# kolinko/effort

Measured on NVIDIA H100. Metric: Mistral-7B decode tok/s @ effort 0.25, higher is better.
Workload: dtype fp16 weights, f32 accumulate

## Files before the change

effort_b200/build.py:

```python
from __future__ import annotations

import os
import shutil
import subprocess

HERE = os.path.dirname(os.path.abspath(__file__))
CSRC = os.path.join(HERE, "csrc")
LIB = os.path.join(HERE, "libeffort_b200.so")
SOURCES = ["effort_capi.cu", "safetensors_io.cpp"]
HEADERS = ["common.cuh", "cutoff.cuh", "bucket_mul.cuh", "convert.cuh", "q4.cuh", "decode.cuh", "comm.cuh"]
NVCC_FLAGS = [
    "-gencode", "arch=compute_90a,code=sm_90a", "-O3", "-lineinfo", "-std=c++17",
    "-Xcompiler", "-fPIC", "-shared",
]


def _nvcc() -> str:
    for cand in (os.environ.get("NVCC"), shutil.which("nvcc"), "/usr/local/cuda/bin/nvcc"):
        if cand and os.path.exists(cand):
            return cand
    raise RuntimeError("nvcc not found: the effort_b200 CUDA extension cannot be built")


def needs_build() -> bool:
    if not os.path.exists(LIB):
        return True
    t = os.path.getmtime(LIB)
    deps = [os.path.join(CSRC, s) for s in SOURCES + HEADERS] + [os.path.join(HERE, "..", "include", "effort_b200.h")]
    return any(os.path.exists(d) and os.path.getmtime(d) > t for d in deps)


def build(force: bool = False, verbose: bool = False) -> str:
    if not force and not needs_build():
        return LIB
    extra = os.environ.get("EFFORT_NVCC_EXTRA", "").split()
    cmd = [_nvcc()] + NVCC_FLAGS + extra + (["-Xptxas", "-v"] if verbose else []) + ["-o", LIB] + \
          [os.path.join(CSRC, s) for s in SOURCES]
    host_cc = "/usr/bin/g++"
    if os.path.exists(host_cc):
        cmd += ["-ccbin", host_cc]
    r = subprocess.run(cmd, capture_output=True, text=True)
    if r.returncode != 0:
        raise RuntimeError("nvcc failed:\n" + r.stdout + r.stderr)
# ... 8 lines not shown
```

effort_b200/csrc/bucket_mul_v2.cuh:

```cuda
#pragma once
#include "bucket_mul.cuh"

namespace effort {

constexpr int kV2Warps = 16;
constexpr int kV2Threads = kV2Warps * 32;
constexpr int kUnitRows = 4;
template <int VEC> struct V2Unit {
    static constexpr int kRowStride = 32 * VEC * 2;
    static constexpr int kUnitBytes = kUnitRows * kRowStride + 32;
};
constexpr int kV2MaxInputs = kV2Threads;

enum VMode : int { kVPlain = 0, kVNorm = 1, kVSilu = 2 };
enum OutMode : int { kOutOverwrite = 0, kOutAccumulate = 1 };
enum CutMode : int { kCutSelect = 0, kCutBisect = 1 };

struct V2Problem {
    const float* v;
    const float* v2;
    const float* v_cut;
    const __half* norm_w;
    const __half* st16;
    const float* st32;
    const uint16_t* bk;
    const __half* probes;
    const uint32_t* exp_no;
    float* out;
    const float* out_scale;
    unsigned* sync;
    uint32_t* sel_counts;
    float* cutoff_out;
    float* cutoff_hint;
    int* rounds_out;
    unsigned* err_flag;
    unsigned long long* trace;
    float4* red_part;
    unsigned* red_sync;
    unsigned long long* unit_trace;
    float norm_eps;
    int in, C, P, q, layout, out_mode;
    int CS, RS, W;
    int R, lpr;
};

struct V2Batch {
    int n;
    int list_cap;
    int dynamic;
    int ring_bytes;
    int prefetch;
    int lookahead;
    int trace_cycles;
    int window;
    int cta_begin[kMulBatchMax + 1];
    V2Problem p[kMulBatchMax];
};

struct V2Header {
    CutoffSmem cut;
    unsigned sel_acc[8][2];
    float red[kV2Warps];
    int warp_cnt[kV2Warps];
    int warp_rows[kV2Warps];
    int next_unit;
};

template <int SLOTS, int VEC>
struct V2Smem {
    static constexpr int kTileFloats = SLOTS * 32 * VEC;
    static constexpr int kTileBytes = kTileFloats * 4;
    static constexpr size_t kHdrBytes = (sizeof(V2Header) + 127) & ~size_t(127);
    static __host__ __device__ size_t list_bytes(int cap) { return ((size_t)cap * 2 + 127) & ~size_t(127); }
    static constexpr size_t kStatBytes = SLOTS == 16 ? 0 : (size_t)kV2MaxInputs * 8 * 4;
    static constexpr int kUnitsPerInput = SLOTS == 16 ? 8 : 4;
    static __host__ __device__ size_t fixed_bytes(int cap) {
        return (size_t)kTileBytes + (size_t)kV2Warps * kTileBytes + kHdrBytes + 2 * (size_t)kV2MaxInputs * 4 + kStatBytes +
               list_bytes(cap) + 128;
    }
    static __host__ __device__ size_t bytes(int cap, int ring_units) {
        return fixed_bytes(cap) + (size_t)kV2Warps * ring_units * V2Unit<VEC>::kUnitBytes;
    }
};

__device__ __forceinline__ void cp_async16(uint32_t dst, const void* src, uint64_t pol) {
    asm volatile("cp.async.cg.shared.global.L2::cache_hint [%0], [%1], 16, %2;" ::"r"(dst), "l"(src), "l"(pol) : "memory");
}
// ... 536 lines not shown
```

effort_b200/csrc/bucket_mul_v4.cuh:

```cuda
#pragma once
#include "bucket_mul_v3.cuh"

namespace effort {

constexpr int kV4Pairs = 8;
constexpr int kV4Units = 16;
constexpr int kV4RingBytes = 16 * 1024;
constexpr int kV4SelWarps = 8;
constexpr int kSelVals = EFFORT_PROBES_MAX / (kV4SelWarps * 32);
constexpr int kSelKeys = kSelVals / 2, kSelChunks = kSelVals / 8;
static_assert(kSelVals * kV4SelWarps * 32 == EFFORT_PROBES_MAX && kSelChunks >= 1, "the group holds all 4096 products");

struct __align__(16) V4Desc {
    uint32_t off;
    uint32_t n;
    float val;
    uint32_t charged;
};

struct V4Header {
    CutoffSmem cut;
    uint2 sel_slot[2][kV4SelWarps];
    float red[kV4SelWarps];
    float cutoff, denom;
    int sel_rows;
    uint32_t warp_rows[kV2Threads / 32];
    uint32_t start[kV4Pairs + 1];
    unsigned long long full_bar[kV4Pairs][kV4Units];
    unsigned long long empty_bar[kV4Pairs][kV4Units];
    V4Desc desc[kV4Pairs][kV4Units];
};

struct V4Smem {
    static constexpr int kTileFloats = 16 * 32 * 4;
    static constexpr int kTileBytes = kTileFloats * 4;
    static constexpr size_t kHdrBytes = (sizeof(V4Header) + 127) & ~size_t(127);
    static constexpr size_t kBytes = (size_t)kTileBytes  + (size_t)kV4Pairs * kTileBytes + kHdrBytes +
                                     (size_t)kV2MaxInputs * 16 + 128 + (size_t)kV4Pairs * kV4RingBytes +
                                     1024 ;
};

__device__ __forceinline__ void cp_async_arrive_noinc(uint32_t bar) {
    asm volatile("cp.async.mbarrier.arrive.noinc.shared::cta.b64 [%0];" ::"r"(bar) : "memory");
}

__device__ __forceinline__ bool mbar_wait_parked(uint32_t bar, uint32_t parity) {
    uint32_t done = 0;
    for (int tries = 0; tries < (1 << 22) && !done; tries++) {
        asm volatile("{ .reg .pred p; mbarrier.try_wait.parity.shared::cta.b64 p, [%1], %2, %3; selp.u32 %0, 1, 0, p; }"
                     : "=r"(done) : "r"(bar), "r"(parity), "r"(200u) : "memory");
    }
    return done != 0;
}

__device__ __forceinline__ bool mbar_test(uint32_t bar, uint32_t parity) {
    uint32_t done;
    asm volatile("{ .reg .pred p; mbarrier.test_wait.parity.shared::cta.b64 p, [%1], %2; selp.u32 %0, 1, 0, p; }"
                 : "=r"(done) : "r"(bar), "r"(parity) : "memory");
    return done != 0;
}

__device__ __forceinline__ float div_by(float x, float d, float r) {
    const float q = x * r;
    return fmaf(fmaf(-q, d, x), r, q);
}

__device__ __forceinline__ uint32_t count_gt32(const uint32_t (&keys)[kSelKeys], uint32_t th) {
    const __nv_bfloat162 t = as_bf162(splat_bf16(th));
    __nv_bfloat162 c0 = __hgt2(as_bf162(keys[0]), t), c1 = __hgt2(as_bf162(keys[1]), t);
#pragma unroll
    for (int i = 2; i < kSelKeys; i += 2) {
        c0 = __hadd2(c0, __hgt2(as_bf162(keys[i]), t));
        c1 = __hadd2(c1, __hgt2(as_bf162(keys[i + 1]), t));
// ... 90 lines not shown
    for (int rho = 0; rho < 16; rho++) sel_stat[rho] = 0.f;
    auto load_stats = [&](int j, float (&st)[16]) {
        const int i = rsp + j * RS;
        if (P == 16) {
            const uint4* sp = reinterpret_cast<const uint4*>(pb.st16 + ((size_t)e_no * pb.in + i) * 16);
            const uint4 a = ldg_keep_u4(sp, keep), b = ldg_keep_u4(sp + 1, keep);
            const uint32_t ws[8] = {a.x, a.y, a.z, a.w, b.x, b.y, b.z, b.w};
#pragma unroll
            for (int q2 = 0; q2 < 8; q2++) {
                const float2 f = __half22float2(*reinterpret_cast<const __half2*>(&ws[q2]));
                st[2 * q2] = f.x;
                st[2 * q2 + 1] = f.y;
            }
        } else {
#pragma unroll
            for (int rho = 0; rho < 16; rho++)
                if (rho < P) st[rho] = __half2float(pb.st16[((size_t)e_no * pb.in + i) * P + rho]);
        }
    };
    if (tid < n_in) load_stats(tid, sel_stat);
    const int vmode = pb.norm_w ? kVNorm : (pb.v2 ? kVSilu : kVPlain);
    uint4 prb[kSelChunks], nwv[kSelChunks];
    if (CUT == kCutSelect && sel_warp) {
        const uint4* pp = reinterpret_cast<const uint4*>(pb.probes + (size_t)e_no * EFFORT_PROBES_MAX) + kSelChunks * tid;
#pragma unroll
        for (int c = 0; c < kSelChunks; c++) prb[c] = ldg_keep_u4(pp + c, keep);
        if (vmode == kVNorm) {
            const uint4* np4 = reinterpret_cast<const uint4*>(pb.norm_w) + kSelChunks * tid;
#pragma unroll
            for (int c = 0; c < kSelChunks; c++) nwv[c] = np4[c];
        }
    }
    if (warp == NC) {
        for (int s = lane; s < NC * kV4Units; s += 32) {
            mbar_init((uint32_t)__cvta_generic_to_shared(&hdr.full_bar[0][0] + s), BULK ? 1 : 33);
            mbar_init((uint32_t)__cvta_generic_to_shared(&hdr.empty_bar[0][0] + s), 1);
        }
        if (lane == 0) hdr.sel_rows = 0;
    }
    const int slice_cols = min(pb.W, C - slice * pb.W);
    const int seg_bytes = slice_cols * 2;
    const bool full_width = slice_cols == TW;
    const int lpr = pb.lpr, R = pb.R;
    const uint32_t base_lane = (tiles_saddr + (uint32_t)pair * V4Smem::kTileBytes) | (uint32_t)(lane * 4);
    const uint64_t pol = l2_policy_evict_first();
    const uint4* bk16 = reinterpret_cast<const uint4*>(pb.bk + (size_t)pb.in * P * ((size_t)slice * pb.W));
    const uint32_t rs16 = (uint32_t)(seg_bytes >> 4);
    auto src_of = [&](int j) { return (uint32_t)(((size_t)e_no * pb.in * P * C + (size_t)(rsp + j * RS) * P * slice_cols) >> 3); };
    const uint32_t my_src0 = src_of(tid);

    unsigned long long* utrace = (pb.unit_trace && blockIdx.x == 0 && pair == 0) ? pb.unit_trace : nullptr;
    if (utrace && tid == 0) utrace[640] = (unsigned long long)clock64();
    uint32_t seq = 0, tail_seq = 0, head = 0, free_b = kV4RingBytes;
    uint32_t slot_charged = 0u;
    const uint32_t full0 = (uint32_t)__cvta_generic_to_shared(&hdr.full_bar[pair][0]);
    const uint32_t empty0 = (uint32_t)__cvta_generic_to_shared(&hdr.empty_bar[pair][0]);
    const uint32_t desc0 = (uint32_t)__cvta_generic_to_shared(&hdr.desc[pair][0]);
    V2_TRACE(1);
    pdl_wait();
    if (cst) cst[1] = (unsigned long long)clock64();

    float my_v = 0.f, my_x3 = 0.f, my_nw = 1.f;
    if (tid < n_in) {
        const int i = rsp + tid * RS;
        my_v = pb.v[i];
        if (vmode == kVSilu) my_x3 = pb.v2[i];
        if (vmode == kVNorm) my_nw = __half2float(pb.norm_w[i]);
    }
    const int seg_bytes0 = slice_cols * 2;
    const uint4* bk16p = reinterpret_cast<const uint4*>(pb.bk + (size_t)pb.in * P * ((size_t)slice * pb.W));
    if (batch.prefetch && pb.cutoff_hint && (CUT != kCutSelect || !sel_warp)) {
        const float hint = pb.cutoff_hint[e_no];
        auto spec = [&](int jj, const float (&st)[16], float vraw) {
            int n = 0;
#pragma unroll
            for (int rho = 0; rho < 16; rho++) n += (rho == n && rho < P && row_selected(hint, st[rho], vraw)) ? 1 : 0;
            if (n > 0) {
                const int i = rsp + jj * RS;
                const uint4* src = bk16p + (((size_t)e_no * pb.in * P * C + (size_t)i * P * slice_cols) >> 3);
                asm volatile("cp.async.bulk.prefetch.L2.global [%0], %1;" ::"l"(src), "r"(n * seg_bytes0) : "memory");
            }
        };
        auto raw = [&](float x, float x3, float nw) { return vmode == kVSilu ? silu_mul(x, x3) : (vmode == kVNorm ? x * nw : x); };
        if (tid < n_in) spec(tid, sel_stat, raw(my_v, my_x3, my_nw));
        if (CUT == kCutSelect && tid >= kV4SelWarps * 32 && tid < 2 * kV4SelWarps * 32 && tid - kV4SelWarps * 32 < n_in) {
            const int j2 = tid - kV4SelWarps * 32;
            float st2[16];
#pragma unroll
            for (int rho = 0; rho < 16; rho++) st2[rho] = 0.f;
            load_stats(j2, st2);
// ... 170 lines not shown
            }
            if (cst && j0 == 0) cst[6] = (unsigned long long)clock64();
            uint32_t incl = len;
#pragma unroll
            for (int o = 1; o < 32; o <<= 1) {
                const uint32_t y = __shfl_up_sync(0xffffffffu, incl, o);
                if (lane >= o) incl += y;
            }
            if (lane == 31) hdr.warp_rows[warp] = incl;
            if (tid <= NC) hdr.start[tid] = tid ? nu_pass : 0u;
            more = __syncthreads_or(m != 0u) != 0;
            uint32_t row_lo, row_hi;
            {
                uint32_t off = 0u, total = 0u;
#pragma unroll
                for (int w = 0; w < NT / 32; w++) {
                    const uint32_t x = hdr.warp_rows[w];
                    total += x;
                    if (w < warp) off += x;
                }
                row_lo = (uint32_t)pair * total / NC;
                row_hi = (uint32_t)(pair + 1) * total / NC;
                if ((uint32_t)tid < nu_pass) {
                    const uint32_t e = off + incl - len;
                    ulist[tid].w = e;
#pragma unroll
                    for (int q = 1; q < NC; q++) {
                        const uint32_t T = (uint32_t)q * total / NC;
                        if (e <= T && T < e + len) hdr.start[q] = (uint32_t)tid;
                    }
                }
                __syncthreads();
            }
            auto clip = [&](uint4 rec) {
                const uint32_t lo = max(rec.w, row_lo), hi = min(rec.w + rec.y, row_hi);
                rec.x += (lo - rec.w) * rs16;
                rec.y = hi > lo ? hi - lo : 0u;
                return rec;
            };
            const uint32_t r_next = hdr.start[pair + 1];
            const uint32_t r_end = r_next < nu_pass ? r_next + 1u : nu_pass;
            if (cst && j0 == 0) cst[7] = (unsigned long long)clock64();
            V2_TRACE(8);

            if (!consumer && BULK) {
                auto reclaim = [&](bool block) {
                    const uint32_t out_n = seq - tail_seq;
                    const uint32_t rel = ((uint32_t)lane - tail_seq) & (kV4Units - 1);
                    const bool mine = lane < kV4Units && rel < out_n;
                    bool done = false;
                    if (mine) {
                        const uint32_t par = ((tail_seq + rel) / kV4Units) & 1u;
                        done = mbar_test(empty0 + (uint32_t)lane * 8u, par);
                        if (block && rel == 0 && !done) {
                            done = mbar_wait_parked(empty0 + (uint32_t)lane * 8u, par);
                            if (!done && pb.err_flag) atomicExch(pb.err_flag, 3u);
                            done = true;
                        }
                    }
                    const unsigned dm = __ballot_sync(0xffffffffu, done) & 0xFFFFu;
                    const unsigned rot = ((dm | (dm << 16)) >> (tail_seq & (kV4Units - 1))) & 0xFFFFu;
                    const uint32_t n = min((uint32_t)(__ffs((int)~rot) - 1), out_n);
                    const uint32_t got = __reduce_add_sync(0xffffffffu, (mine && rel < n) ? slot_charged : 0u);
                    free_b += got;
                    tail_seq += n;
                };
                uint32_t t0 = hdr.start[pair], grabs = 0u;
#pragma unroll 1
                for (; t0 < r_end; t0 += min(min((uint32_t)batch.window, grabs), r_end - t0)) {
                    grabs++;
                    const uint32_t cnt = min(min((uint32_t)batch.window, grabs), r_end - t0);
                    uint4 rec = make_uint4(0u, 0u, 0u, 0u);
                    if ((uint32_t)lane < cnt) rec = clip(ulist[t0 + lane]);
                    const uint32_t my_bytes = rec.y * (uint32_t)seg_bytes;
                    uint32_t pos = 0u;
                    if (seq != tail_seq) reclaim(false);
#pragma unroll 1
                    while (pos < cnt) {
                        uint32_t h = head, f = free_b, n_ok = 0u, n_seen = 0u, my_off = 0u, my_chg = 0u, my_k = 0xffffffffu;
                        const uint32_t slots_free = (uint32_t)kV4Units - (seq - tail_seq);
                        for (uint32_t l = pos; l < cnt; l++) {
                            const uint32_t bts = __shfl_sync(0xffffffffu, my_bytes, (int)l);
                            if (bts == 0u) { n_seen++; continue; }
                            const uint32_t skip = (h + bts > (uint32_t)kV4RingBytes) ? ((uint32_t)kV4RingBytes - h) : 0u;
                            if (f < bts + skip || n_ok >= slots_free) break;
                            const uint32_t off = skip ? 0u : h;
                            if ((uint32_t)lane == l) { my_off = off; my_chg = bts + skip; my_k = n_ok; }
                            if ((uint32_t)lane == ((seq + n_ok) & (kV4Units - 1))) slot_charged = bts + skip;
                            h = off + bts;
                            if (h >= (uint32_t)kV4RingBytes) h = 0u;
                            f -= bts + skip;
                            n_ok++;
                            n_seen++;
                        }
                        if (n_seen == 0u) { reclaim(true); continue; }
                        if (my_k != 0xffffffffu) {
                            const uint32_t slot = (seq + my_k) & (kV4Units - 1);
                            const uint32_t fb = full0 + slot * 8u;
                            asm volatile("st.shared.v4.u32 [%0], {%1,%2,%3,%4};" ::"r"(desc0 + slot * 16u), "r"(my_off), "r"(rec.y), "r"(rec.z),
                                         "r"(my_chg) : "memory");
                            if (utrace && seq + my_k < 80u) { utrace[8 * (seq + my_k)] = (unsigned long long)clock64(); utrace[8 * (seq + my_k) + 3] = (unsigned long long)rec.y; }
                            mbar_expect_tx(fb, (int)my_bytes);
                            bulk_g2s(ring_saddr + my_off, bk16 + rec.x, (int)my_bytes, fb, pol);
                        }
                        seq += n_ok;
                        head = h;
                        free_b = f;
                        pos += n_seen;
                    }
                }
                while (seq - tail_seq >= (uint32_t)kV4Units) reclaim(true);
                {
                    const uint32_t slot = seq & (kV4Units - 1);
                    if (lane == 0) {
                        asm volatile("st.shared.v4.u32 [%0], {%1,%2,%3,%4};" ::"r"(desc0 + slot * 16u), "r"(0u), "r"(0u), "r"(0u), "r"(0u) : "memory");
                        mbar_arrive(full0 + slot * 8u);
                    }
                    if ((uint32_t)lane == slot) slot_charged = 0u;
                    seq++;
                }
            } else if (!consumer) {
                auto reclaim = [&]() {
                    const uint32_t ts = tail_seq & (kV4Units - 1);
                    if (!mbar_wait_parked(empty0 + ts * 8u, (tail_seq / kV4Units) & 1u)) {
                        if (pb.err_flag && lane == 0) atomicExch(pb.err_flag, 3u);
                    }
                    free_b += hdr.desc[pair][ts].charged;
                    tail_seq++;
                };
                auto fill = [&](uint32_t src16, uint32_t len, uint32_t valbits) {
                    const uint32_t bytes = len * (uint32_t)seg_bytes;
                    const uint32_t skip = (head + bytes > (uint32_t)kV4RingBytes) ? ((uint32_t)kV4RingBytes - head) : 0u;
                    while (free_b < bytes + skip || seq - tail_seq >= (uint32_t)kV4Units) reclaim();
                    const uint32_t off = skip ? 0u : head;
                    const uint32_t slot = seq & (kV4Units - 1);
                    const uint32_t sa = ring_saddr + off;
                    const uint32_t fb = full0 + slot * 8u;
                    const uint4* src = bk16 + src16;
                    if (lane == 0)
                        asm volatile("st.shared.v4.u32 [%0], {%1,%2,%3,%4};" ::"r"(desc0 + slot * 16u), "r"(off), "r"(len), "r"(valbits),
                                     "r"(bytes + skip) : "memory");
                    if (utrace && lane == 0 && seq < 80u) { utrace[8 * seq] = (unsigned long long)clock64(); utrace[8 * seq + 3] = (unsigned long long)len; }
                    const uint32_t pieces = len * rs16;
                    const uint32_t d0 = sa + (uint32_t)lane * 16u;
                    const uint4* s0p = src + lane;
                    for (uint32_t q = (uint32_t)lane; q < pieces; q += 32u) cp_async16(d0 + (q - (uint32_t)lane) * 16u, s0p + (q - (uint32_t)lane), pol);
                    cp_async_arrive_noinc(fb);
                    __syncwarp();
                    if (lane == 0) mbar_arrive(fb);
                    seq++;
                    head = off + bytes;
                    free_b -= bytes + skip;
                    if (head >= (uint32_t)kV4RingBytes) head = 0u;
                };
#pragma unroll 1
                for (uint32_t t = hdr.start[pair]; t < r_end; t++) {
                    const uint4 rec = clip(ulist[t]);
                    if (rec.y != 0u) fill(rec.x, rec.y, rec.z);
                }
                fill(0u, 0u, 0u);
            } else {
                unsigned long long rows_done = 0ull;
                bool nx_ok = false;
                uint32_t nx_off = 0u, nx_n = 0u, nx_val = 0u;
#pragma unroll 1
                for (;;) {
                    const uint32_t slot = seq & (kV4Units - 1);
                    uint32_t hoff, hn, hv, hs;
                    if (utrace && lane == 0 && seq < 80u) utrace[8 * seq + 1] = (unsigned long long)clock64();
                    if (nx_ok) {
                        hoff = nx_off; hn = nx_n; hv = nx_val;
                    } else {
                        if (!mbar_wait(full0 + slot * 8u, (seq / kV4Units) & 1u)) {
                            if (pb.err_flag && lane == 0) atomicExch(pb.err_flag, 2u);
                            break;
                        }
                        asm volatile("ld.shared.v4.u32 {%0,%1,%2,%3}, [%4];" : "=r"(hoff), "=r"(hn), "=r"(hv), "=r"(hs) : "r"(desc0 + slot * 16u));
                    }
                    if (utrace && lane == 0 && seq < 80u) utrace[8 * seq + 2] = (unsigned long long)clock64();
                    seq++;
                    nx_ok = false;
                    if (batch.lookahead && hn != 0u) {
                        const uint32_t nslot = seq & (kV4Units - 1);
                        nx_ok = mbar_test(full0 + nslot * 8u, (seq / kV4Units) & 1u);
                        if (nx_ok)
                            asm volatile("ld.shared.v4.u32 {%0,%1,%2,%3}, [%4];" : "=r"(nx_off), "=r"(nx_n), "=r"(nx_val), "=r"(hs) : "r"(desc0 + nslot * 16u));
                    }
                    const int n = (int)hn;
                    if (utrace && lane == 0 && seq <= 80u && n >= 0) utrace[8 * (seq - 1) + 4] = (unsigned long long)clock64();
                    const uint32_t eb = empty0 + slot * 8u;
                    if (n == 0) {
                        if (lane == 0) mbar_arrive(eb);
                        break;
                    }
                    rows_done += (unsigned long long)n;
                    const float val = __uint_as_float(hv);
                    const uint32_t sa = ring_saddr + hoff;
                    if (full_width) {
                        uint32_t a0 = sa + (uint32_t)(lane * LB);
                        int r = 0;
                        for (; r + 4 <= n; r += 4, a0 += 4 * kRow) {
                            accumulate_unit_fp16<VEC, 4, kRow>(base_lane, val, a0);
                            if (utrace && lane == 0 && seq <= 80u && r == 0) utrace[8 * (seq - 1) + 5] = (unsigned long long)clock64();
                        }
                        switch (n - r) {
                            case 1: accumulate_unit_fp16<VEC, 1, kRow>(base_lane, val, a0); break;
                            case 2: accumulate_unit_fp16<VEC, 2, kRow>(base_lane, val, a0); break;
                            case 3: accumulate_unit_fp16<VEC, 3, kRow>(base_lane, val, a0); break;
                            default: break;
                        }
                    } else {
                        const int rowslot = lane / lpr, lcol = lane % lpr;
                        const bool col_ok = lcol * VEC < slice_cols;
                        for (int st = 0; st * R < n; st++) {
                            const int r = st * R + rowslot;
                            const bool ok = (rowslot < R) && (r < n) && col_ok;
                            uint32_t ww[2] = {0u, 0u};
                            if (ok) asm volatile("ld.shared.v2.u32 {%0,%1}, [%2];" : "=r"(ww[0]), "=r"(ww[1]) : "r"(sa + (uint32_t)(r * seg_bytes + lcol * LB)));
                            accumulate_words<SLOTS, VEC>(base_lane, ok ? val : 0.f, ww);
                        }
                    }
                    if (utrace && lane == 0 && seq <= 80u) utrace[8 * (seq - 1) + 6] = (unsigned long long)clock64();
                    __syncwarp();
                    if (lane == 0) mbar_arrive(eb);
                    if (utrace && lane == 0 && seq <= 80u) utrace[8 * (seq - 1) + 7] = (unsigned long long)clock64();
                }
                if (lane == 0 && rows_done) atomicAdd(&hdr.sel_rows, (int)rows_done);
                if (pb.unit_trace && blockIdx.x == 0 && lane == 0) {
                    unsigned long long* fin = pb.unit_trace + 648;
                    fin[warp] = (unsigned long long)clock64();
                    fin[16 + warp] = rows_done;
                    fin[32 + warp] = (unsigned long long)seq;
                }
            }
        } while (more);
    }
    __syncthreads();
    if (pb.sel_counts && slice == 0 && tid == 0) pb.sel_counts[rsp] = (uint32_t)hdr.sel_rows;
    V2_TRACE(9);
    if (cst) cst[8] = (unsigned long long)clock64();

    {
        constexpr int NG = NT / TW, SPT = SLOTS / NG;
        static_assert(SPT == 4, "one 16-byte reduction per thread");
        const int cl = tid % TW, sg = tid / TW;
        const int k = cl >> 5, ln = cl & 31;
        float acc[SPT] = {0.f, 0.f, 0.f, 0.f};
        const bool col_on = (ln < lpr) && (ln * VEC + k < slice_cols);
        if (col_on) {
            for (int rs2 = 0; rs2 < R; rs2++) {
                const int word0 = (sg * SPT) * TW + k * 32 + ln + rs2 * lpr;
#pragma unroll
                for (int w = 0; w < NC; w++)
#pragma unroll
                    for (int s = 0; s < SPT; s++) acc[s] += tiles[(size_t)w * TF + word0 + s * TW];
            }
        }
        pb.red_part[(size_t)blockIdx.x * NT + tid] = make_float4(acc[0], acc[1], acc[2], acc[3]);
// ... 54 lines not shown
```

effort_b200/csrc/effort_capi.cu:

```cuda
#include "../../include/effort_b200.h"

#include <atomic>
#include <cstdio>
#include <cstdlib>
#include <cstring>
#include <map>
#include <new>
#include <string>
#include <utility>
#include <vector>

#include "bucket_mul.cuh"
#include "bucket_mul_v2.cuh"
#include "bucket_mul_v3.cuh"
#include "bucket_mul_v4.cuh"
#include "comm.cuh"
#include "convert.cuh"
#include "cutoff.cuh"
#include "q4.cuh"

using namespace effort;

static std::atomic<uint64_t> g_launches{0};
static thread_local std::string g_cuda_err;
// ... 28 lines not shown
    __half* st16 = nullptr;
    float* st32 = nullptr;
    float* hint = nullptr;
    size_t owned = 0;
    int layout = kInputMajor;
    int device = 0;
    const uint16_t* fast_bk() const { return bk_own ? bk_own : buckets; }
};

struct effort_ctx {
    int device = 0;
    int n_sms = 0;
    float* cutoff = nullptr;
    int* loops = nullptr;
    uint32_t* sizes = nullptr;
    float2* dispatch = nullptr;
    size_t dispatch_cap = 0;
    uint32_t* chunk_counts = nullptr;
    size_t chunk_cap = 0;
    float* partial = nullptr;
    size_t partial_cap = 0;
    uint32_t* sel_counts = nullptr;
    size_t sel_cap = 0;
    bool have_dispatch = false;
    int dispatch_kind = 0;
    unsigned long long* trace = nullptr;
    unsigned* v2_sync = nullptr;
    unsigned* v2_err = nullptr;
    float4* v4_part = nullptr;
    unsigned* v4_sync = nullptr;
    int cutoff_mode = 0;
    int stage_mode = 4;
    int engine = 2;
    int lookahead = 1;
    int window = 8;
    int prefetch = 0;
    int use_hint = 1;
    int dynamic = 0;
    int last_rs[8] = {0};
    bool last_was_v2 = false;
    void* comm = nullptr;
    int comm_rank = 0, comm_world = 1;
    unsigned char* p2p_local = nullptr;
    void* p2p_peer[16] = {nullptr};
    bool p2p_ready = false;
};

static constexpr int kMaxBatch = 8;
static constexpr int kV2MaxSlices = 64;

static bool default_slice_major();

extern "C" int effort_version(void) { return EFFORT_B200_VERSION; }
extern "C" const char* effort_last_cuda_error(void) { return g_cuda_err.c_str(); }
extern "C" uint64_t effort_launch_count(void) { return g_launches.load(); }

extern "C" const char* effort_strerror(int code) {
    switch (code) {
        case EFFORT_OK: return "ok";
        case EFFORT_EINVAL: return "invalid argument / reference precondition failed";
        case EFFORT_ECUDA: return "CUDA runtime error";
        case EFFORT_ENOMEM: return "out of memory";
        case EFFORT_ESHAPE: return "shape not supported by the kernels";
        case EFFORT_ESTATE: return "call sequence error";
        case EFFORT_ENOTLOADED: return "buckets not loaded and no dense core";
        default: return "unknown error";
    }
}
// ... 1 lines not shown
extern "C" int effort_ctx_create(int device, effort_ctx_t** ctx_out) {
    if (!ctx_out) return EFFORT_EINVAL;
    *ctx_out = nullptr;
    int dev = device;
    if (dev < 0) CK(cudaGetDevice(&dev));
    else CK(cudaSetDevice(dev));
    effort_ctx* c = new (std::nothrow) effort_ctx();
    if (!c) return EFFORT_ENOMEM;
    c->device = dev;
    cudaDeviceProp prop;
    CK(cudaGetDeviceProperties(&prop, dev));
    c->n_sms = prop.multiProcessorCount;
    CK(cudaMalloc(&c->cutoff, sizeof(float) * kMaxBatch));
    CK(cudaMalloc(&c->loops, sizeof(int)));
    CK(cudaMalloc(&c->sizes, sizeof(uint32_t) * (4 + kMaxBatch)));
    CK(cudaMemset(c->sizes, 0, sizeof(uint32_t) * (4 + kMaxBatch)));
    CK(cudaMemset(c->cutoff, 0, sizeof(float) * kMaxBatch));
    CK(cudaMemset(c->loops, 0, sizeof(int)));
    CK(cudaMalloc(&c->v2_sync, sizeof(unsigned) * kMaxBatch * kV2MaxSlices * 2));
    CK(cudaMemset(c->v2_sync, 0, sizeof(unsigned) * kMaxBatch * kV2MaxSlices * 2));
    CK(cudaMalloc(&c->v4_part, sizeof(float4) * kV2Threads * c->n_sms));
    CK(cudaMalloc(&c->v4_sync, sizeof(unsigned) * kMaxBatch * kV2MaxSlices * 2));
    CK(cudaMemset(c->v4_sync, 0, sizeof(unsigned) * kMaxBatch * kV2MaxSlices * 2));
    CK(cudaMalloc(&c->v2_err, sizeof(unsigned)));
    CK(cudaMemset(c->v2_err, 0, sizeof(unsigned)));
    CK(cudaMalloc(&c->sel_counts, sizeof(uint32_t) * kMaxBatch * c->n_sms));
    CK(cudaMemset(c->sel_counts, 0, sizeof(uint32_t) * kMaxBatch * c->n_sms));
    c->sel_cap = (size_t)kMaxBatch * c->n_sms;
    { const char* e = getenv("EFFORT_CUTOFF"); if (e && !strcmp(e, "bisect")) c->cutoff_mode = 1; }
    { const char* e = getenv("EFFORT_STAGE"); if (e) c->stage_mode = !strcmp(e, "ldgsts") ? 0 : !strcmp(e, "tma") ? 2 : !strcmp(e, "pairs-ldgsts") ? 3 : 4; }
    { const char* e = getenv("EFFORT_ENGINE"); if (e && atoi(e) == 1) c->engine = 1; }
    { const char* e = getenv("EFFORT_DYN"); if (e) c->dynamic = atoi(e) ? 1 : 0; }
    { const char* e = getenv("EFFORT_PREFETCH"); if (e) c->prefetch = atoi(e) ? 1 : 0; }
    { const char* e = getenv("EFFORT_LOOKAHEAD"); if (e) c->lookahead = atoi(e) ? 1 : 0; }
    { const char* e = getenv("EFFORT_WINDOW"); if (e && atoi(e) >= 1 && atoi(e) <= 8) c->window = atoi(e); }
    { const char* e = getenv("EFFORT_HINT"); if (e) c->use_hint = atoi(e) ? 1 : 0; }
    if (getenv("EFFORT_TRACE")) {
        CK(cudaMalloc(&c->trace, sizeof(unsigned long long) * (16 * c->n_sms + 648 + 48 + 16)));
        CK(cudaMemset(c->trace, 0, sizeof(unsigned long long) * (16 * c->n_sms + 648 + 48 + 16)));
    }
    *ctx_out = c;
    return EFFORT_OK;
}

extern "C" int effort_ctx_set_cutoff_mode(effort_ctx_t* c, int mode) {
    if (!c || (mode != EFFORT_CUTOFF_SELECT && mode != EFFORT_CUTOFF_BISECT)) return EFFORT_EINVAL;
    c->cutoff_mode = mode;
    return EFFORT_OK;
}

extern "C" int effort_ctx_set_option(effort_ctx_t* c, const char* name, int value) {
    if (!c || !name) return EFFORT_EINVAL;
    if (!strcmp(name, "engine")) { if (value != 1 && value != 2) return EFFORT_EINVAL; c->engine = value; return EFFORT_OK; }
    if (!strcmp(name, "stage")) { if (value != 0 && value != 2 && value != 3 && value != 4) return EFFORT_EINVAL; c->stage_mode = value; return EFFORT_OK; }
    if (!strcmp(name, "hint")) { if (value != 0 && value != 1) return EFFORT_EINVAL; c->use_hint = value; return EFFORT_OK; }
    if (!strcmp(name, "lookahead")) { if (value != 0 && value != 1) return EFFORT_EINVAL; c->lookahead = value; return EFFORT_OK; }
    if (!strcmp(name, "window")) { if (value < 1 || value > 8) return EFFORT_EINVAL; c->window = value; return EFFORT_OK; }
    if (!strcmp(name, "prefetch")) { if (value != 0 && value != 1) return EFFORT_EINVAL; c->prefetch = value; return EFFORT_OK; }
    if (!strcmp(name, "dynamic")) { if (value != 0 && value != 1) return EFFORT_EINVAL; c->dynamic = value; return EFFORT_OK; }
    return EFFORT_EINVAL;
}

extern "C" int effort_ctx_error_flag(effort_ctx_t* c, unsigned* flag_out, void* stream) {
    if (!c || !flag_out) return EFFORT_EINVAL;
    CK(cudaStreamSynchronize((cudaStream_t)stream));
    CK(cudaMemcpy(flag_out, c->v2_err, sizeof(unsigned), cudaMemcpyDeviceToHost));
    return EFFORT_OK;
}

extern "C" int effort_debug_read_unit_trace(effort_ctx_t* c, unsigned long long* host648) {
    if (!c || !c->trace || !host648) return EFFORT_EINVAL;
    CK(cudaDeviceSynchronize());
    CK(cudaMemcpy(host648, c->trace + 16 * c->n_sms, sizeof(unsigned long long) * (648 + 48 + 16), cudaMemcpyDeviceToHost));
    CK(cudaMemset(c->trace + 16 * c->n_sms, 0, sizeof(unsigned long long) * (648 + 48 + 16)));
    return EFFORT_OK;
}

extern "C" int effort_debug_read_trace(effort_ctx_t* c, unsigned long long* host, int max_rows) {
    if (!c || !c->trace || !host) return EFFORT_EINVAL;
    CK(cudaDeviceSynchronize());
    int n = c->n_sms < max_rows ? c->n_sms : max_rows;
    CK(cudaMemcpy(host, c->trace, sizeof(unsigned long long) * 16 * n, cudaMemcpyDeviceToHost));
    return n;
}

extern "C" int effort_ctx_destroy(effort_ctx_t* c) {
    if (!c) return EFFORT_OK;
    cudaFree(c->cutoff); cudaFree(c->loops); cudaFree(c->sizes); cudaFree(c->dispatch);
    cudaFree(c->chunk_counts); cudaFree(c->partial); cudaFree(c->sel_counts);
    cudaFree(c->trace); cudaFree(c->v2_sync); cudaFree(c->v2_err); cudaFree(c->v4_part); cudaFree(c->v4_sync);
// ... 288 lines not shown
        if (norm && silu) return EFFORT_EINVAL;
        if ((norm || silu) && c.v_cut) return EFFORT_EINVAL;
        if (norm && w->in != 8 * kV2Threads) return EFFORT_ESHAPE;
        if (!c.v_cut && w->in < EFFORT_PROBES_MAX) return EFFORT_ESHAPE;
        pb.v = c.v; pb.v2 = c.v2; pb.v_cut = c.v_cut ? c.v_cut : c.v; pb.norm_w = c.norm_w; pb.norm_eps = c.norm_eps;
        pb.st16 = w->st16; pb.st32 = w->st32; pb.bk = w->fast_bk(); pb.probes = w->probes; pb.exp_no = c.exp_no;
        pb.out = c.out; pb.out_scale = c.out_scale;
        pb.sync = ctx->v2_sync + (size_t)(slot0 + k) * kV2MaxSlices * 2;
        pb.red_sync = ctx->v4_sync + (size_t)(slot0 + k) * kV2MaxSlices * 2;
        pb.red_part = ctx->v4_part;
        pb.sel_counts = ctx->sel_counts + (size_t)(slot0 + k) * ctx->n_sms;
        pb.cutoff_out = ctx->cutoff + slot0 + k;
        pb.cutoff_hint = ctx->use_hint ? w->hint : nullptr;
        pb.rounds_out = (slot0 + k == 0) ? ctx->loops : nullptr;
        pb.err_flag = ctx->v2_err;
        pb.trace = ctx->trace;
        pb.unit_trace = ctx->trace ? ctx->trace + 16 * ctx->n_sms : nullptr;
        pb.in = w->in; pb.C = w->C; pb.P = w->P; pb.q = effort_q(c.effort, w->n_probes); pb.layout = w->layout;
        pb.out_mode = c.out_mode;
        pb.CS = g.CS; pb.RS = rs; pb.W = (g.CS == 1) ? w->C : 32 * VEC; pb.R = g.R; pb.lpr = g.lpr;
        const int per_cta = (w->in + rs - 1) / rs;
        const int cap = (per_cta < kV2MaxInputs ? per_cta : kV2MaxInputs) * V2Smem<SLOTS, VEC>::kUnitsPerInput;
        list_cap = cap > list_cap ? cap : list_cap;
        batch.cta_begin[k] = cta;
        cta += g.CS * rs;
        ctx->last_rs[slot0 + k] = rs;
    }
    if (cta > n_cta) return EFFORT_ESHAPE;
    batch.cta_begin[n] = cta;
    batch.list_cap = (list_cap + 63) & ~63;
    using L = V2Smem<SLOTS, VEC>;
    batch.dynamic = ctx->dynamic;
    batch.prefetch = ctx->prefetch;
    batch.window = ctx->window;
    { static const int tc = [] { const char* e = getenv("EFFORT_TRACE"); return e && atoi(e) == 2 ? 1 : 0; }(); batch.trace_cycles = tc; }
    batch.lookahead = ctx->lookahead;
    const size_t smem = L::bytes(batch.list_cap, D);
    if (smem > kMaxSmem) return EFFORT_ESHAPE;
    auto go = [&](void (*kernel)(const V2Batch), int threads, size_t smem_bytes) -> int {
        static std::map<std::pair<int, const void*>, bool> configured;
        const auto key = std::make_pair(ctx->device, (const void*)kernel);
        if (!configured.count(key)) {
            cudaFuncAttributes fa{};
            CK(cudaFuncGetAttributes(&fa, kernel));
            CK(cudaFuncSetAttribute(kernel, cudaFuncAttributeMaxDynamicSharedMemorySize, (int)(kMaxSmem - fa.sharedSizeBytes)));
            configured[key] = true;
        }
        CK(launch_pdl(kernel, dim3(cta), dim3(threads), smem_bytes, stream, batch));
        return EFFORT_OK;
    };
    int rc;
    const bool bisect = ctx->cutoff_mode == 1;
    bool all_slice = true;
    for (int k = 0; k < n; k++) all_slice = all_slice && calls[k].w->layout == kSliceMajor;
    if (SLOTS == 16 && all_slice && ctx->stage_mode == 3) {
        rc = bisect ? go(bucket_mul_v4_kernel<kCutBisect, false>, kV2Threads, V4Smem::kBytes)
                    : go(bucket_mul_v4_kernel<kCutSelect, false>, kV2Threads, V4Smem::kBytes);
    } else if (SLOTS == 16 && all_slice && ctx->stage_mode == 4) {
        rc = bisect ? go(bucket_mul_v4_kernel<kCutBisect, true>, kV2Threads, V4Smem::kBytes)
                    : go(bucket_mul_v4_kernel<kCutSelect, true>, kV2Threads, V4Smem::kBytes);
    } else if (SLOTS == 16 && all_slice && ctx->stage_mode == 2) {
        batch.ring_bytes = (int)((kMaxSmem - V3Smem::kFixed) & ~(size_t)255);
        if (batch.ring_bytes < 2 * (kV3BatchBytes + 4096)) return EFFORT_ESHAPE;
        const size_t smem3 = V3Smem::kFixed + (size_t)batch.ring_bytes;
        rc = bisect ? go(bucket_mul_v3_kernel<kCutBisect>, kV3Threads, smem3) : go(bucket_mul_v3_kernel<kCutSelect>, kV3Threads, smem3);
    } else if (bisect) {
        rc = go(bucket_mul_v2_kernel<SLOTS, VEC, kCutBisect, D>, kV2Threads, smem);
    } else {
        rc = go(bucket_mul_v2_kernel<SLOTS, VEC, kCutSelect, D>, kV2Threads, smem);
// ... 1037 lines not shown
```

Measured before the change: 252.4.

## Replace per-unit descriptor ring with fixed row-chunk slots in v4 bucket mul

The v4 producer/consumer pipeline used a variable-size byte ring with per-unit descriptors, a grab window and consumer lookahead. It now uses fixed 16-row chunks (4 slots × 4 KB per pair), and producer and consumer both walk the unit list independently to map row pieces into chunk slots. This cuts descriptor traffic, per-unit barrier handshakes and ring accounting, and lets several small units share one barrier wait. The cost is that units straddling chunks are split into several copies, chunk granularity can leave slots partly used, and the window and lookahead knobs are removed.

```diff
diff --git a/effort_b200/build.py b/effort_b200/build.py
--- a/effort_b200/build.py
+++ b/effort_b200/build.py
@@ -8,7 +8,8 @@
 CSRC = os.path.join(HERE, "csrc")
 LIB = os.path.join(HERE, "libeffort_b200.so")
 SOURCES = ["effort_capi.cu", "safetensors_io.cpp"]
-HEADERS = ["common.cuh", "cutoff.cuh", "bucket_mul.cuh", "convert.cuh", "q4.cuh", "decode.cuh", "comm.cuh"]
+HEADERS = ["common.cuh", "cutoff.cuh", "bucket_mul.cuh", "bucket_mul_v2.cuh", "bucket_mul_v3.cuh", "bucket_mul_v4.cuh",
+           "convert.cuh", "q4.cuh", "decode.cuh", "comm.cuh"]
 NVCC_FLAGS = [
     "-gencode", "arch=compute_90a,code=sm_90a", "-O3", "-lineinfo", "-std=c++17",
     "-Xcompiler", "-fPIC", "-shared",
diff --git a/effort_b200/csrc/bucket_mul_v2.cuh b/effort_b200/csrc/bucket_mul_v2.cuh
--- a/effort_b200/csrc/bucket_mul_v2.cuh
+++ b/effort_b200/csrc/bucket_mul_v2.cuh
@@ -50,9 +50,7 @@
     int dynamic;
     int ring_bytes;
     int prefetch;
-    int lookahead;
     int trace_cycles;
-    int window;
     int cta_begin[kMulBatchMax + 1];
     V2Problem p[kMulBatchMax];
 };
diff --git a/effort_b200/csrc/bucket_mul_v4.cuh b/effort_b200/csrc/bucket_mul_v4.cuh
--- a/effort_b200/csrc/bucket_mul_v4.cuh
+++ b/effort_b200/csrc/bucket_mul_v4.cuh
@@ -4,19 +4,14 @@
 namespace effort {
 
 constexpr int kV4Pairs = 8;
-constexpr int kV4Units = 16;
-constexpr int kV4RingBytes = 16 * 1024;
+constexpr int kV4Chunks = 4;
+constexpr int kV4ChunkRows = 16;
+constexpr int kV4ChunkBytes = kV4ChunkRows * 256;
+constexpr int kV4RingBytes = kV4Chunks * kV4ChunkBytes;
 constexpr int kV4SelWarps = 8;
 constexpr int kSelVals = EFFORT_PROBES_MAX / (kV4SelWarps * 32);
 constexpr int kSelKeys = kSelVals / 2, kSelChunks = kSelVals / 8;
 static_assert(kSelVals * kV4SelWarps * 32 == EFFORT_PROBES_MAX && kSelChunks >= 1, "the group holds all 4096 products");
-
-struct __align__(16) V4Desc {
-    uint32_t off;
-    uint32_t n;
-    float val;
-    uint32_t charged;
-};
 
 struct V4Header {
     CutoffSmem cut;
@@ -26,9 +21,8 @@
     int sel_rows;
     uint32_t warp_rows[kV2Threads / 32];
     uint32_t start[kV4Pairs + 1];
-    unsigned long long full_bar[kV4Pairs][kV4Units];
-    unsigned long long empty_bar[kV4Pairs][kV4Units];
-    V4Desc desc[kV4Pairs][kV4Units];
+    unsigned long long full_bar[kV4Pairs][kV4Chunks];
+    unsigned long long empty_bar[kV4Pairs][kV4Chunks];
 };
 
 struct V4Smem {
@@ -39,6 +33,23 @@
                                      (size_t)kV2MaxInputs * 16 + 128 + (size_t)kV4Pairs * kV4RingBytes +
                                      1024 ;
 };
+
+__device__ __forceinline__ uint32_t v4_slot(uint32_t s) { return s & (kV4Chunks - 1); }
+__device__ __forceinline__ uint32_t v4_phase(uint32_t s) { return (s / kV4Chunks) & 1u; }
+
+struct V4Piece {
+    uint32_t lo, hi;
+    uint4 rec;
+};
+__device__ __forceinline__ uint32_t v4_pieces(const uint4* ulist, uint32_t t, uint32_t r_end, uint32_t c0, uint32_t c1, int lane,
+                                              V4Piece& pc) {
+    const bool have = t + (uint32_t)lane < r_end;
+    pc.rec = have ? ulist[t + lane] : make_uint4(0u, 0u, 0u, 0u);
+    pc.lo = max(pc.rec.w, c0);
+    pc.hi = min(pc.rec.w + pc.rec.y, c1);
+    const unsigned fin = __ballot_sync(0xffffffffu, have && pc.rec.w + pc.rec.y <= c1);
+    return fin == 0xffffffffu ? 32u : (uint32_t)(__ffs((int)~fin) - 1);
+}
 
 __device__ __forceinline__ void cp_async_arrive_noinc(uint32_t bar) {
     asm volatile("cp.async.mbarrier.arrive.noinc.shared::cta.b64 [%0];" ::"r"(bar) : "memory");
@@ -195,8 +206,8 @@
         }
     }
     if (warp == NC) {
-        for (int s = lane; s < NC * kV4Units; s += 32) {
-            mbar_init((uint32_t)__cvta_generic_to_shared(&hdr.full_bar[0][0] + s), BULK ? 1 : 33);
+        for (int s = lane; s < NC * kV4Chunks; s += 32) {
+            mbar_init((uint32_t)__cvta_generic_to_shared(&hdr.full_bar[0][0] + s), BULK ? 1 : 32);
             mbar_init((uint32_t)__cvta_generic_to_shared(&hdr.empty_bar[0][0] + s), 1);
         }
         if (lane == 0) hdr.sel_rows = 0;
@@ -214,11 +225,9 @@
 
     unsigned long long* utrace = (pb.unit_trace && blockIdx.x == 0 && pair == 0) ? pb.unit_trace : nullptr;
     if (utrace && tid == 0) utrace[640] = (unsigned long long)clock64();
-    uint32_t seq = 0, tail_seq = 0, head = 0, free_b = kV4RingBytes;
-    uint32_t slot_charged = 0u;
+    uint32_t seq = 0;
     const uint32_t full0 = (uint32_t)__cvta_generic_to_shared(&hdr.full_bar[pair][0]);
     const uint32_t empty0 = (uint32_t)__cvta_generic_to_shared(&hdr.empty_bar[pair][0]);
-    const uint32_t desc0 = (uint32_t)__cvta_generic_to_shared(&hdr.desc[pair][0]);
     V2_TRACE(1);
     pdl_wait();
     if (cst) cst[1] = (unsigned long long)clock64();
@@ -455,198 +464,144 @@
                 }
                 __syncthreads();
             }
-            auto clip = [&](uint4 rec) {
-                const uint32_t lo = max(rec.w, row_lo), hi = min(rec.w + rec.y, row_hi);
-                rec.x += (lo - rec.w) * rs16;
-                rec.y = hi > lo ? hi - lo : 0u;
-                return rec;
-            };
             const uint32_t r_next = hdr.start[pair + 1];
             const uint32_t r_end = r_next < nu_pass ? r_next + 1u : nu_pass;
+            const uint32_t kb = row_lo / (uint32_t)kV4ChunkRows;
+            const uint32_t n_chunks = row_hi > row_lo ? (row_hi - 1u) / (uint32_t)kV4ChunkRows + 1u - kb : 0u;
+            auto chunk_lo = [&](uint32_t c) { return max((kb + c) * (uint32_t)kV4ChunkRows, row_lo); };
+            auto chunk_hi = [&](uint32_t c) { return min((kb + c + 1u) * (uint32_t)kV4ChunkRows, row_hi); };
+            auto chunk_of = [&](uint32_t r) { return r / (uint32_t)kV4ChunkRows - kb; };
+            auto at = [&](uint32_t r) { return (r % (uint32_t)kV4ChunkRows) * (uint32_t)seg_bytes; };
+            const uint32_t seq0 = seq;
+            seq += n_chunks;
             if (cst && j0 == 0) cst[7] = (unsigned long long)clock64();
             V2_TRACE(8);
 
-            if (!consumer && BULK) {
-                auto reclaim = [&](bool block) {
-                    const uint32_t out_n = seq - tail_seq;
-                    const uint32_t rel = ((uint32_t)lane - tail_seq) & (kV4Units - 1);
-                    const bool mine = lane < kV4Units && rel < out_n;
-                    bool done = false;
-                    if (mine) {
-                        const uint32_t par = ((tail_seq + rel) / kV4Units) & 1u;
-                        done = mbar_test(empty0 + (uint32_t)lane * 8u, par);
-                        if (block && rel == 0 && !done) {
-                            done = mbar_wait_parked(empty0 + (uint32_t)lane * 8u, par);
-                            if (!done && pb.err_flag) atomicExch(pb.err_flag, 3u);
-                            done = true;
+            if (!consumer) {
+                uint32_t t = hdr.start[pair];
+#pragma unroll 1
+                for (uint32_t c = 0; c < n_chunks;) {
+                    const uint32_t s = seq0 + c + (uint32_t)lane;
+                    const bool free_slot = lane < kV4Chunks && c + (uint32_t)lane < n_chunks &&
+                                           (s < (uint32_t)kV4Chunks || mbar_test(empty0 + v4_slot(s) * 8u, v4_phase(s) ^ 1u));
+                    uint32_t k = (uint32_t)(__ffs((int)~__ballot_sync(0xffffffffu, free_slot)) - 1);
+                    if (k == 0u) {
+                        const uint32_t so = seq0 + c;
+                        if (!mbar_wait_parked(empty0 + v4_slot(so) * 8u, v4_phase(so) ^ 1u) && pb.err_flag && lane == 0)
+                            atomicExch(pb.err_flag, 3u);
+                        k = 1u;
+                    }
+                    if ((uint32_t)lane < k) {
+                        const uint32_t cc = c + (uint32_t)lane;
+                        if (BULK) mbar_expect_tx(full0 + v4_slot(seq0 + cc) * 8u, (int)((chunk_hi(cc) - chunk_lo(cc)) * (uint32_t)seg_bytes));
+                        if (utrace && seq0 + cc < 80u) {
+                            utrace[8 * (seq0 + cc)] = (unsigned long long)clock64();
+                            utrace[8 * (seq0 + cc) + 3] = (unsigned long long)(chunk_hi(cc) - chunk_lo(cc));
                         }
                     }
-                    const unsigned dm = __ballot_sync(0xffffffffu, done) & 0xFFFFu;
-                    const unsigned rot = ((dm | (dm << 16)) >> (tail_seq & (kV4Units - 1))) & 0xFFFFu;
-                    const uint32_t n = min((uint32_t)(__ffs((int)~rot) - 1), out_n);
-                    const uint32_t got = __reduce_add_sync(0xffffffffu, (mine && rel < n) ? slot_charged : 0u);
-                    free_b += got;
-                    tail_seq += n;
-                };
-                uint32_t t0 = hdr.start[pair], grabs = 0u;
+                    __syncwarp();
+                    const uint32_t b0 = chunk_lo(c), b1 = chunk_hi(c + k - 1u);
 #pragma unroll 1
-                for (; t0 < r_end; t0 += min(min((uint32_t)batch.window, grabs), r_end - t0)) {
-                    grabs++;
-                    const uint32_t cnt = min(min((uint32_t)batch.window, grabs), r_end - t0);
-                    uint4 rec = make_uint4(0u, 0u, 0u, 0u);
-                    if ((uint32_t)lane < cnt) rec = clip(ulist[t0 + lane]);
-                    const uint32_t my_bytes = rec.y * (uint32_t)seg_bytes;
-                    uint32_t pos = 0u;
-                    if (seq != tail_seq) reclaim(false);
-#pragma unroll 1
-                    while (pos < cnt) {
-                        uint32_t h = head, f = free_b, n_ok = 0u, n_seen = 0u, my_off = 0u, my_chg = 0u, my_k = 0xffffffffu;
-                        const uint32_t slots_free = (uint32_t)kV4Units - (seq - tail_seq);
-                        for (uint32_t l = pos; l < cnt; l++) {
-                            const uint32_t bts = __shfl_sync(0xffffffffu, my_bytes, (int)l);
-                            if (bts == 0u) { n_seen++; continue; }
-                            const uint32_t skip = (h + bts > (uint32_t)kV4RingBytes) ? ((uint32_t)kV4RingBytes - h) : 0u;
-                            if (f < bts + skip || n_ok >= slots_free) break;
-                            const uint32_t off = skip ? 0u : h;
-                            if ((uint32_t)lane == l) { my_off = off; my_chg = bts + skip; my_k = n_ok; }
-                            if ((uint32_t)lane == ((seq + n_ok) & (kV4Units - 1))) slot_charged = bts + skip;
-                            h = off + bts;
-                            if (h >= (uint32_t)kV4RingBytes) h = 0u;
-                            f -= bts + skip;
-                            n_ok++;
-                            n_seen++;
+                    for (;;) {
+                        V4Piece pc;
+                        const uint32_t done = v4_pieces(ulist, t, r_end, b0, b1, lane, pc);
+                        if (BULK) {
+                            for (uint32_t lo = pc.lo; lo < pc.hi;) {
+                                const uint32_t cc = chunk_of(lo), sl = v4_slot(seq0 + cc);
+                                const uint32_t hi = min(pc.hi, chunk_hi(cc));
+                                bulk_g2s(ring_saddr + sl * (uint32_t)kV4ChunkBytes + at(lo),
+                                         bk16 + pc.rec.x + (lo - pc.rec.w) * rs16, (int)((hi - lo) * (uint32_t)seg_bytes), full0 + sl * 8u, pol);
+                                lo = hi;
+                            }
+                        } else {
+                            unsigned todo = __ballot_sync(0xffffffffu, pc.lo < pc.hi);
+                            while (todo) {
+                                const int l = __ffs((int)todo) - 1;
+                                todo &= todo - 1u;
+                                uint32_t lo = __shfl_sync(0xffffffffu, pc.lo, l);
+                                const uint32_t phi = __shfl_sync(0xffffffffu, pc.hi, l);
+                                uint32_t src = __shfl_sync(0xffffffffu, pc.rec.x, l) + (lo - __shfl_sync(0xffffffffu, pc.rec.w, l)) * rs16;
+                                while (lo < phi) {
+                                    const uint32_t cc = chunk_of(lo);
+                                    const uint32_t hi = min(phi, chunk_hi(cc));
+                                    const uint32_t d0 = ring_saddr + v4_slot(seq0 + cc) * (uint32_t)kV4ChunkBytes + at(lo);
+                                    const uint32_t n16 = (hi - lo) * rs16;
+                                    for (uint32_t q = (uint32_t)lane; q < n16; q += 32u) cp_async16(d0 + q * 16u, bk16 + src + q, pol);
+                                    src += n16;
+                                    lo = hi;
+                                }
+                            }
                         }
-                        if (n_seen == 0u) { reclaim(true); continue; }
-                        if (my_k != 0xffffffffu) {
-                            const uint32_t slot = (seq + my_k) & (kV4Units - 1);
-                            const uint32_t fb = full0 + slot * 8u;
-                            asm volatile("st.shared.v4.u32 [%0], {%1,%2,%3,%4};" ::"r"(desc0 + slot * 16u), "r"(my_off), "r"(rec.y), "r"(rec.z),
-                                         "r"(my_chg) : "memory");
-                            if (utrace && seq + my_k < 80u) { utrace[8 * (seq + my_k)] = (unsigned long long)clock64(); utrace[8 * (seq + my_k) + 3] = (unsigned long long)rec.y; }
-                            mbar_expect_tx(fb, (int)my_bytes);
-                            bulk_g2s(ring_saddr + my_off, bk16 + rec.x, (int)my_bytes, fb, pol);
-                        }
-                        seq += n_ok;
-                        head = h;
-                        free_b = f;
-                        pos += n_seen;
-                    }
-                }
-                while (seq - tail_seq >= (uint32_t)kV4Units) reclaim(true);
-                {
-                    const uint32_t slot = seq & (kV4Units - 1);
-                    if (lane == 0) {
-                        asm volatile("st.shared.v4.u32 [%0], {%1,%2,%3,%4};" ::"r"(desc0 + slot * 16u), "r"(0u), "r"(0u), "r"(0u), "r"(0u) : "memory");
-                        mbar_arrive(full0 + slot * 8u);
-                    }
-                    if ((uint32_t)lane == slot) slot_charged = 0u;
-                    seq++;
-                }
-            } else if (!consumer) {
-                auto reclaim = [&]() {
-                    const uint32_t ts = tail_seq & (kV4Units - 1);
-                    if (!mbar_wait_parked(empty0 + ts * 8u, (tail_seq / kV4Units) & 1u)) {
-                        if (pb.err_flag && lane == 0) atomicExch(pb.err_flag, 3u);
-                    }
-                    free_b += hdr.desc[pair][ts].charged;
-                    tail_seq++;
-                };
-                auto fill = [&](uint32_t src16, uint32_t len, uint32_t valbits) {
-                    const uint32_t bytes = len * (uint32_t)seg_bytes;
-                    const uint32_t skip = (head + bytes > (uint32_t)kV4RingBytes) ? ((uint32_t)kV4RingBytes - head) : 0u;
-                    while (free_b < bytes + skip || seq - tail_seq >= (uint32_t)kV4Units) reclaim();
-                    const uint32_t off = skip ? 0u : head;
-                    const uint32_t slot = seq & (kV4Units - 1);
-                    const uint32_t sa = ring_saddr + off;
-                    const uint32_t fb = full0 + slot * 8u;
-                    const uint4* src = bk16 + src16;
-                    if (lane == 0)
-                        asm volatile("st.shared.v4.u32 [%0], {%1,%2,%3,%4};" ::"r"(desc0 + slot * 16u), "r"(off), "r"(len), "r"(valbits),
-                                     "r"(bytes + skip) : "memory");
-                    if (utrace && lane == 0 && seq < 80u) { utrace[8 * seq] = (unsigned long long)clock64(); utrace[8 * seq + 3] = (unsigned long long)len; }
-                    const uint32_t pieces = len * rs16;
-                    const uint32_t d0 = sa + (uint32_t)lane * 16u;
-                    const uint4* s0p = src + lane;
-                    for (uint32_t q = (uint32_t)lane; q < pieces; q += 32u) cp_async16(d0 + (q - (uint32_t)lane) * 16u, s0p + (q - (uint32_t)lane), pol);
-                    cp_async_arrive_noinc(fb);
-                    __syncwarp();
-                    if (lane == 0) mbar_arrive(fb);
-                    seq++;
-                    head = off + bytes;
-                    free_b -= bytes + skip;
-                    if (head >= (uint32_t)kV4RingBytes) head = 0u;
-                };
-#pragma unroll 1
-                for (uint32_t t = hdr.start[pair]; t < r_end; t++) {
-                    const uint4 rec = clip(ulist[t]);
-                    if (rec.y != 0u) fill(rec.x, rec.y, rec.z);
-                }
-                fill(0u, 0u, 0u);
+                        t += done;
+                        if (done < 32u) break;
+                    }
+                    if (!BULK)
+                        for (uint32_t i = 0; i < k; i++) cp_async_arrive_noinc(full0 + v4_slot(seq0 + c + i) * 8u);
+                    c += k;
+                }
             } else {
                 unsigned long long rows_done = 0ull;
-                bool nx_ok = false;
-                uint32_t nx_off = 0u, nx_n = 0u, nx_val = 0u;
+                uint32_t t = hdr.start[pair];
 #pragma unroll 1
-                for (;;) {
-                    const uint32_t slot = seq & (kV4Units - 1);
-                    uint32_t hoff, hn, hv, hs;
-                    if (utrace && lane == 0 && seq < 80u) utrace[8 * seq + 1] = (unsigned long long)clock64();
-                    if (nx_ok) {
-                        hoff = nx_off; hn = nx_n; hv = nx_val;
-                    } else {
-                        if (!mbar_wait(full0 + slot * 8u, (seq / kV4Units) & 1u)) {
-                            if (pb.err_flag && lane == 0) atomicExch(pb.err_flag, 2u);
-                            break;
+                for (uint32_t c = 0; c < n_chunks; c++) {
+                    const uint32_t s = seq0 + c, sl = v4_slot(s);
+                    const uint32_t c0 = chunk_lo(c), c1 = chunk_hi(c);
+                    const bool tr = utrace && lane == 0 && s < 80u;
+                    if (tr) utrace[8 * s + 1] = (unsigned long long)clock64();
+                    V4Piece pc;
+                    uint32_t done = v4_pieces(ulist, t, r_end, c0, c1, lane, pc);
+                    if (!mbar_wait(full0 + sl * 8u, v4_phase(s))) {
+                        if (pb.err_flag && lane == 0) atomicExch(pb.err_flag, 2u);
+                        break;
+                    }
+                    if (tr) utrace[8 * s + 2] = (unsigned long long)clock64();
+                    if (tr) utrace[8 * s + 4] = (unsigned long long)clock64();
+                    const uint32_t cbase = ring_saddr + sl * (uint32_t)kV4ChunkBytes;
+                    bool first = true;
+#pragma unroll 1
+                    for (;;) {
+                        unsigned todo = __ballot_sync(0xffffffffu, pc.lo < pc.hi);
+                        while (todo) {
+                            const int l = __ffs((int)todo) - 1;
+                            todo &= todo - 1u;
+                            const uint32_t lo = __shfl_sync(0xffffffffu, pc.lo, l);
+                            const int n = (int)(__shfl_sync(0xffffffffu, pc.hi, l) - lo);
+                            const float val = __uint_as_float(__shfl_sync(0xffffffffu, pc.rec.z, l));
+                            const uint32_t sa = cbase + at(lo);
+                            if (full_width) {
+                                uint32_t a0 = sa + (uint32_t)(lane * LB);
+                                int r = 0;
+                                for (; r + 4 <= n; r += 4, a0 += 4 * kRow) accumulate_unit_fp16<VEC, 4, kRow>(base_lane, val, a0);
+                                switch (n - r) {
+                                    case 1: accumulate_unit_fp16<VEC, 1, kRow>(base_lane, val, a0); break;
+                                    case 2: accumulate_unit_fp16<VEC, 2, kRow>(base_lane, val, a0); break;
+                                    case 3: accumulate_unit_fp16<VEC, 3, kRow>(base_lane, val, a0); break;
+                                    default: break;
+                                }
+                            } else {
+                                const int rowslot = lane / lpr, lcol = lane % lpr;
+                                const bool col_ok = lcol * VEC < slice_cols;
+                                const int k0 = (int)(lo - max(__shfl_sync(0xffffffffu, pc.rec.w, l), row_lo));
+                                for (int st = k0 / R; st * R < k0 + n; st++) {
+                                    const int r = st * R + rowslot;
+                                    const bool ok = (rowslot < R) && (r >= k0) && (r < k0 + n) && col_ok;
+                                    uint32_t ww[2] = {0u, 0u};
+                                    if (ok) asm volatile("ld.shared.v2.u32 {%0,%1}, [%2];" : "=r"(ww[0]), "=r"(ww[1]) : "r"(sa + (uint32_t)((r - k0) * seg_bytes + lcol * LB)));
+                                    accumulate_words<SLOTS, VEC>(base_lane, ok ? val : 0.f, ww);
+                                }
+                            }
+                            if (tr && first) utrace[8 * s + 5] = (unsigned long long)clock64();
+                            first = false;
                         }
-                        asm volatile("ld.shared.v4.u32 {%0,%1,%2,%3}, [%4];" : "=r"(hoff), "=r"(hn), "=r"(hv), "=r"(hs) : "r"(desc0 + slot * 16u));
-                    }
-                    if (utrace && lane == 0 && seq < 80u) utrace[8 * seq + 2] = (unsigned long long)clock64();
-                    seq++;
-                    nx_ok = false;
-                    if (batch.lookahead && hn != 0u) {
-                        const uint32_t nslot = seq & (kV4Units - 1);
-                        nx_ok = mbar_test(full0 + nslot * 8u, (seq / kV4Units) & 1u);
-                        if (nx_ok)
-                            asm volatile("ld.shared.v4.u32 {%0,%1,%2,%3}, [%4];" : "=r"(nx_off), "=r"(nx_n), "=r"(nx_val), "=r"(hs) : "r"(desc0 + nslot * 16u));
-                    }
-                    const int n = (int)hn;
-                    if (utrace && lane == 0 && seq <= 80u && n >= 0) utrace[8 * (seq - 1) + 4] = (unsigned long long)clock64();
-                    const uint32_t eb = empty0 + slot * 8u;
-                    if (n == 0) {
-                        if (lane == 0) mbar_arrive(eb);
-                        break;
-                    }
-                    rows_done += (unsigned long long)n;
-                    const float val = __uint_as_float(hv);
-                    const uint32_t sa = ring_saddr + hoff;
-                    if (full_width) {
-                        uint32_t a0 = sa + (uint32_t)(lane * LB);
-                        int r = 0;
-                        for (; r + 4 <= n; r += 4, a0 += 4 * kRow) {
-                            accumulate_unit_fp16<VEC, 4, kRow>(base_lane, val, a0);
-                            if (utrace && lane == 0 && seq <= 80u && r == 0) utrace[8 * (seq - 1) + 5] = (unsigned long long)clock64();
-                        }
-                        switch (n - r) {
-                            case 1: accumulate_unit_fp16<VEC, 1, kRow>(base_lane, val, a0); break;
-                            case 2: accumulate_unit_fp16<VEC, 2, kRow>(base_lane, val, a0); break;
-                            case 3: accumulate_unit_fp16<VEC, 3, kRow>(base_lane, val, a0); break;
-                            default: break;
-                        }
-                    } else {
-                        const int rowslot = lane / lpr, lcol = lane % lpr;
-                        const bool col_ok = lcol * VEC < slice_cols;
-                        for (int st = 0; st * R < n; st++) {
-                            const int r = st * R + rowslot;
-                            const bool ok = (rowslot < R) && (r < n) && col_ok;
-                            uint32_t ww[2] = {0u, 0u};
-                            if (ok) asm volatile("ld.shared.v2.u32 {%0,%1}, [%2];" : "=r"(ww[0]), "=r"(ww[1]) : "r"(sa + (uint32_t)(r * seg_bytes + lcol * LB)));
-                            accumulate_words<SLOTS, VEC>(base_lane, ok ? val : 0.f, ww);
-                        }
-                    }
-                    if (utrace && lane == 0 && seq <= 80u) utrace[8 * (seq - 1) + 6] = (unsigned long long)clock64();
+                        t += done;
+                        if (done < 32u) break;
+                        done = v4_pieces(ulist, t, r_end, c0, c1, lane, pc);
+                    }
+                    rows_done += (unsigned long long)(c1 - c0);
+                    if (tr) utrace[8 * s + 6] = (unsigned long long)clock64();
                     __syncwarp();
-                    if (lane == 0) mbar_arrive(eb);
-                    if (utrace && lane == 0 && seq <= 80u) utrace[8 * (seq - 1) + 7] = (unsigned long long)clock64();
+                    if (lane == 0) mbar_arrive(empty0 + sl * 8u);
+                    if (tr) utrace[8 * s + 7] = (unsigned long long)clock64();
                 }
                 if (lane == 0 && rows_done) atomicAdd(&hdr.sel_rows, (int)rows_done);
                 if (pb.unit_trace && blockIdx.x == 0 && lane == 0) {
diff --git a/effort_b200/csrc/effort_capi.cu b/effort_b200/csrc/effort_capi.cu
--- a/effort_b200/csrc/effort_capi.cu
+++ b/effort_b200/csrc/effort_capi.cu
@@ -84,8 +84,6 @@
     int cutoff_mode = 0;
     int stage_mode = 4;
     int engine = 2;
-    int lookahead = 1;
-    int window = 8;
     int prefetch = 0;
     int use_hint = 1;
     int dynamic = 0;
@@ -153,8 +151,6 @@
     { const char* e = getenv("EFFORT_ENGINE"); if (e && atoi(e) == 1) c->engine = 1; }
     { const char* e = getenv("EFFORT_DYN"); if (e) c->dynamic = atoi(e) ? 1 : 0; }
     { const char* e = getenv("EFFORT_PREFETCH"); if (e) c->prefetch = atoi(e) ? 1 : 0; }
-    { const char* e = getenv("EFFORT_LOOKAHEAD"); if (e) c->lookahead = atoi(e) ? 1 : 0; }
-    { const char* e = getenv("EFFORT_WINDOW"); if (e && atoi(e) >= 1 && atoi(e) <= 8) c->window = atoi(e); }
     { const char* e = getenv("EFFORT_HINT"); if (e) c->use_hint = atoi(e) ? 1 : 0; }
     if (getenv("EFFORT_TRACE")) {
         CK(cudaMalloc(&c->trace, sizeof(unsigned long long) * (16 * c->n_sms + 648 + 48 + 16)));
@@ -175,8 +171,6 @@
     if (!strcmp(name, "engine")) { if (value != 1 && value != 2) return EFFORT_EINVAL; c->engine = value; return EFFORT_OK; }
     if (!strcmp(name, "stage")) { if (value != 0 && value != 2 && value != 3 && value != 4) return EFFORT_EINVAL; c->stage_mode = value; return EFFORT_OK; }
     if (!strcmp(name, "hint")) { if (value != 0 && value != 1) return EFFORT_EINVAL; c->use_hint = value; return EFFORT_OK; }
-    if (!strcmp(name, "lookahead")) { if (value != 0 && value != 1) return EFFORT_EINVAL; c->lookahead = value; return EFFORT_OK; }
-    if (!strcmp(name, "window")) { if (value < 1 || value > 8) return EFFORT_EINVAL; c->window = value; return EFFORT_OK; }
     if (!strcmp(name, "prefetch")) { if (value != 0 && value != 1) return EFFORT_EINVAL; c->prefetch = value; return EFFORT_OK; }
     if (!strcmp(name, "dynamic")) { if (value != 0 && value != 1) return EFFORT_EINVAL; c->dynamic = value; return EFFORT_OK; }
     return EFFORT_EINVAL;
@@ -531,9 +525,7 @@
     using L = V2Smem<SLOTS, VEC>;
     batch.dynamic = ctx->dynamic;
     batch.prefetch = ctx->prefetch;
-    batch.window = ctx->window;
     { static const int tc = [] { const char* e = getenv("EFFORT_TRACE"); return e && atoi(e) == 2 ? 1 : 0; }(); batch.trace_cycles = tc; }
-    batch.lookahead = ctx->lookahead;
     const size_t smem = L::bytes(batch.list_cap, D);
     if (smem > kMaxSmem) return EFFORT_ESHAPE;
     auto go = [&](void (*kernel)(const V2Batch), int threads, size_t smem_bytes) -> int {
```

After: 275.0, median of 6. 9.0% higher.
